# Yusheng-Xu/VGS-SVGS-Segmentation

Measured on AMD Instinct MI355X. Metric: segmented points/sec (end-to-end VGS), higher is better.
Workload: dtype f32

## Files before the change

include/vgs.h:

```cpp
#ifndef VGS_H_
#define VGS_H_

#include <stdint.h>

#ifdef __cplusplus
extern "C" {
#endif

typedef enum {
  VGS_OK = 0,
  VGS_E_ARG = 1,
  VGS_E_STATE = 2,
  VGS_E_HIP = 3,
  VGS_E_NOMEM = 4,
  VGS_E_UNSUPPORTED = 5,
  VGS_E_IO = 6,
  VGS_E_PEER = 7
} vgs_status;

typedef struct {
  int32_t method;
  float voxel_size;
  float graph_size;
  float sig_p, sig_n, sig_o, sig_e, sig_c, sig_w;
// ... 55 lines not shown
vgs_status vgs_adjacency(vgs_ctx* ctx);
vgs_status vgs_segment(vgs_ctx* ctx);
vgs_status vgs_run(vgs_ctx* ctx);

vgs_status svgs_set_supervoxel_labels(vgs_ctx* ctx, const int32_t* labels_host, int32_t max_label);
vgs_status svgs_supervoxels(vgs_ctx* ctx);
vgs_status svgs_segment(vgs_ctx* ctx);
vgs_status svgs_get_supervoxel_labels(vgs_ctx* ctx, int32_t* labels, int32_t* max_label);

vgs_status vgs_get_counts(vgs_ctx* ctx, int64_t* counts );
vgs_status vgs_get_stage_times(vgs_ctx* ctx, double* ms );
vgs_status vgs_get_schedule_counters(vgs_ctx* ctx, int64_t* out );
vgs_status vgs_get_schedule_counters_ex(vgs_ctx* ctx, int64_t* out, int32_t n);
vgs_status vgs_screen_table(const vgs_params* params, float* d2_stop, float* ctab_scale, float* ctab );
vgs_status vgs_get_bbox(vgs_ctx* ctx, double* min3_max3);
vgs_status vgs_get_voxel_table(vgs_ctx* ctx, uint32_t* key, int32_t* start, int32_t* point_idx);
vgs_status vgs_get_voxel_centers(vgs_ctx* ctx, float* center3V);
vgs_status vgs_get_point_voxel(vgs_ctx* ctx, int32_t* voxel_of_point );
vgs_status vgs_get_attributes(vgs_ctx* ctx, float* centroid, float* normal, float* eigen8, uint8_t* used);
vgs_status vgs_get_lists(vgs_ctx* ctx, int32_t which, int64_t* offsets, int32_t* idx);
enum { VGS_ORDER_VOXEL_ID = 0, VGS_ORDER_REFERENCE = 1 };
vgs_status vgs_get_lists_ordered(vgs_ctx* ctx, int32_t which, int32_t order, int64_t* offsets, int32_t* idx);
vgs_status vgs_get_adjacency_counts(vgs_ctx* ctx, int32_t* n_all );
vgs_status vgs_get_local_weights(vgs_ctx* ctx, int32_t node_id, int32_t* n, int32_t* ids, float* weights);
vgs_status vgs_get_node_labels(vgs_ctx* ctx, int32_t* component_root ,
                               int32_t* kept_label );
vgs_status vgs_get_point_labels(vgs_ctx* ctx, int32_t* labels );
vgs_status vgs_get_point_labels_async(vgs_ctx* ctx, int32_t* labels);
vgs_status vgs_wait_point_labels(vgs_ctx* ctx);
vgs_status vgs_get_point_labels_device(vgs_ctx* ctx, const int32_t** labels_dev );
vgs_status vgs_get_clusters(vgs_ctx* ctx, int64_t* offsets, int32_t* point_idx);
vgs_status vgs_get_clusters_ordered(vgs_ctx* ctx, int32_t order, int64_t* offsets, int32_t* point_idx);
vgs_status vgs_get_clusters_device(vgs_ctx* ctx, const int64_t** offsets_dev, const int32_t** point_idx_dev);
vgs_status vgs_get_segment_descriptors(vgs_ctx* ctx, int64_t* n_points, int32_t* n_nodes, float* bbox6, double* centroid3, double* cov6,
                                       double* evals3, double* evecs9, float* eigen8);
vgs_status vgs_get_segment_descriptors_device(vgs_ctx* ctx, const int64_t** n_points, const int32_t** n_nodes, const float** bbox6,
                                              const double** centroid3, const double** cov6, const double** evals3, const double** evecs9,
                                              const float** eigen8);
vgs_status vgs_get_own_segment_moments(vgs_ctx* ctx, int64_t K, int64_t* n_records, int32_t* label, int64_t* n_points, int32_t* n_nodes,
                                       float* bbox6, float* anchor3, double* s9);
vgs_status vgs_segment_descriptors_from_moments(vgs_ctx* ctx, int64_t K, const int64_t* n_points, const int32_t* n_nodes, const float* bbox6,
                                                const float* anchor3, const double* s9, int64_t* n_points_out, int32_t* n_nodes_out,
                                                float* bbox6_out, double* centroid3, double* cov6, double* evals3, double* evecs9, float* eigen8);
enum { VGS_BOX_PRINCIPAL = 0, VGS_BOX_UPRIGHT = 1 };
vgs_status vgs_get_segment_boxes(vgs_ctx* ctx, int32_t frame, double* center3, double* half3, double* frame9, double* lo3, double* hi3);
vgs_status vgs_get_segment_boxes_device(vgs_ctx* ctx, int32_t frame, const double** center3, const double** half3, const double** frame9,
// ... 35 lines not shown
```

vgs-svgs-segmentation_amd/_lib.py:

```python
from __future__ import annotations

import ctypes as C
import os
import subprocess

_HERE = os.path.dirname(os.path.abspath(__file__))
LIB_PATH = os.path.join(_HERE, os.path.basename(os.environ.get("VGS_LIB", "libvgs_hip.so")))
CSRC = os.path.join(_HERE, "csrc")

VGS_OK, VGS_E_ARG, VGS_E_STATE, VGS_E_HIP, VGS_E_NOMEM, VGS_E_UNSUPPORTED, VGS_E_IO, VGS_E_PEER = range(8)
STATUS_NAMES = ["VGS_OK", "VGS_E_ARG", "VGS_E_STATE", "VGS_E_HIP", "VGS_E_NOMEM", "VGS_E_UNSUPPORTED", "VGS_E_IO", "VGS_E_PEER"]

N_POINTS, N_FINITE, N_VOXELS, N_USED, N_ADJ, N_CLUSTERS, N_KEPT, N_PAIRS, N_DEPTH, N_ISOLATED, N_REATTACHED, N_SUPERVOXELS = range(12)
N_COUNTS = 16
T_VOXELIZE, T_FEATURES, T_ADJACENCY, T_LOCALCUT, T_MERGE, T_LABELS, T_TOTAL, T_LOCALCUT_KERNEL, T_SUPERVOXEL = range(9)
T_COUNT = 12


class VgsParams(C.Structure):
    _fields_ = [
        ("method", C.c_int32), ("voxel_size", C.c_float), ("graph_size", C.c_float),
        ("sig_p", C.c_float), ("sig_n", C.c_float), ("sig_o", C.c_float), ("sig_e", C.c_float), ("sig_c", C.c_float),
        ("sig_w", C.c_float), ("cut_thred", C.c_float),
        ("points_min", C.c_int32), ("adjacency_min", C.c_int32), ("voxels_min", C.c_int32),
# ... 31 lines not shown
    ("vgs_host_unregister", C.c_int, [_P]),
    ("vgs_voxelize", C.c_int, [_P]),
    ("vgs_features", C.c_int, [_P]),
    ("vgs_adjacency", C.c_int, [_P]),
    ("vgs_segment", C.c_int, [_P]),
    ("vgs_run", C.c_int, [_P]),
    ("svgs_set_supervoxel_labels", C.c_int, [_P, _P, C.c_int32]),
    ("svgs_supervoxels", C.c_int, [_P]),
    ("svgs_segment", C.c_int, [_P]),
    ("svgs_get_supervoxel_labels", C.c_int, [_P, _P, C.POINTER(C.c_int32)]),
    ("vgs_get_counts", C.c_int, [_P, _P]),
    ("vgs_get_schedule_counters", C.c_int, [_P, _P]),
    ("vgs_get_schedule_counters_ex", C.c_int, [_P, _P, C.c_int32]),
    ("vgs_screen_table", C.c_int, [_P, _P, _P, _P]),
    ("vgs_get_stage_times", C.c_int, [_P, _P]),
    ("vgs_get_bbox", C.c_int, [_P, _P]),
    ("vgs_get_voxel_table", C.c_int, [_P, _P, _P, _P]),
    ("vgs_get_voxel_centers", C.c_int, [_P, _P]),
    ("vgs_get_point_voxel", C.c_int, [_P, _P]),
    ("vgs_get_attributes", C.c_int, [_P, _P, _P, _P, _P]),
    ("vgs_get_lists", C.c_int, [_P, C.c_int32, _P, _P]),
    ("vgs_get_lists_ordered", C.c_int, [_P, C.c_int32, C.c_int32, _P, _P]),
    ("vgs_get_adjacency_counts", C.c_int, [_P, _P]),
    ("vgs_get_local_weights", C.c_int, [_P, C.c_int32, C.POINTER(C.c_int32), _P, _P]),
    ("vgs_get_node_labels", C.c_int, [_P, _P, _P]),
    ("vgs_get_point_labels", C.c_int, [_P, _P]),
    ("vgs_get_point_labels_async", C.c_int, [_P, _P]),
    ("vgs_wait_point_labels", C.c_int, [_P]),
    ("vgs_get_point_labels_device", C.c_int, [_P, C.POINTER(_P)]),
    ("vgs_get_clusters", C.c_int, [_P, _P, _P]),
    ("vgs_get_clusters_ordered", C.c_int, [_P, C.c_int32, _P, _P]),
    ("vgs_get_clusters_device", C.c_int, [_P, _P, _P]),
    ("vgs_get_segment_descriptors", C.c_int, [_P, _P, _P, _P, _P, _P, _P, _P, _P]),
    ("vgs_get_segment_descriptors_device", C.c_int, [_P, _P, _P, _P, _P, _P, _P, _P, _P]),
    ("vgs_get_own_segment_moments", C.c_int, [_P, C.c_int64, _P, _P, _P, _P, _P, _P, _P]),
    ("vgs_segment_descriptors_from_moments", C.c_int, [_P, C.c_int64, _P, _P, _P, _P, _P, _P, _P, _P, _P, _P, _P, _P, _P]),
    ("vgs_get_segment_boxes", C.c_int, [_P, C.c_int32, _P, _P, _P, _P, _P]),
    ("vgs_get_segment_boxes_device", C.c_int, [_P, C.c_int32, _P, _P, _P, _P, _P]),
    ("vgs_get_own_segment_extents", C.c_int, [_P, C.c_int64, C.c_int32, _P, _P, _P, _P, _P, _P, _P]),
    ("vgs_segment_boxes_from_extents", C.c_int, [_P, C.c_int64, C.c_int32, _P, _P, _P, _P, _P, _P, _P, _P]),
    ("vgs_get_segment_graph", C.c_int, [_P, _P, _P, _P, _P, _P, _P, _P, _P]),
    ("vgs_get_segment_graph_device", C.c_int, [_P, _P, _P, _P, _P, _P, _P, _P, _P]),
    ("vgs_set_halo_labels", C.c_int, [_P, _P, _P, C.c_int64]),
    ("vgs_get_own_segment_graph", C.c_int, [_P, C.c_int64, _P, _P, _P, _P, _P, _P, _P, _P]),
    ("vgs_grid_state_init", C.c_int, [C.POINTER(VgsGridState)]),
    ("vgs_grid_advance", C.c_int, [_P, C.POINTER(VgsGridState)]),
# ... 38 lines not shown
```

vgs-svgs-segmentation_amd/api.py:

```python
from __future__ import annotations

import ctypes as C

import numpy as np

from . import _lib
from ._lib import VgsError, VgsGridState, VgsParams


def default_params(method=2, **kw):
    p = VgsParams()
    L = _lib.lib()
    (L.vgs_params_default_svgs if method == 3 else L.vgs_params_default_vgs)(C.byref(p))
    for k, v in kw.items():
        if not hasattr(p, k):
            raise AttributeError(k)
        setattr(p, k, v)
    return p


def parse_task_file(path):
    p = VgsParams()
    a = C.create_string_buffer(512)
    b = C.create_string_buffer(512)
# ... 142 lines not shown
        cen = np.zeros((V, 3), dtype=np.float32)
        nrm = np.zeros((V, 3), dtype=np.float32)
        eig = np.zeros((V, 8), dtype=np.float32)
        used = np.zeros(V, dtype=np.uint8)
        self._ck(self._L.vgs_get_attributes(self._h, _ptr(cen), _ptr(nrm), _ptr(eig), _ptr(used)))
        return dict(centroid=cen, normal=nrm, eigen=eig, used=used)

    LISTS = {"adjacency": 0, "connect_cut": 1, "connect_cross": 2, "connect_final": 3}

    def lists(self, which, order="voxel_id"):
        V = self.counts()["voxels"]
        off = np.zeros(V + 1, dtype=np.int64)
        w, o = self.LISTS[which], self.ORDERS[order]
        self._ck(self._L.vgs_get_lists_ordered(self._h, w, o, _ptr(off), None))
        idx = np.zeros(max(int(off[-1]), 1), dtype=np.int32)
        self._ck(self._L.vgs_get_lists_ordered(self._h, w, o, _ptr(off), _ptr(idx)))
        return off, idx[:int(off[-1])]

    def adjacency_counts(self):
        out = np.zeros(self.counts()["voxels"], dtype=np.int32)
        self._ck(self._L.vgs_get_adjacency_counts(self._h, _ptr(out)))
        return out

    def local_weights(self, node_id):
        n = C.c_int32(0)
        self._ck(self._L.vgs_get_local_weights(self._h, int(node_id), C.byref(n), None, None))
        ids = np.zeros(max(n.value, 1), dtype=np.int32)
        W = np.zeros((max(n.value, 1), max(n.value, 1)), dtype=np.float32)
        if n.value:
            self._ck(self._L.vgs_get_local_weights(self._h, int(node_id), C.byref(n), _ptr(ids), _ptr(W)))
        return ids[:n.value], W[:n.value, :n.value]

    def node_labels(self):
        V = self.counts()["voxels"]
        root = np.zeros(V, dtype=np.int32)
        kept = np.zeros(V, dtype=np.int32)
        self._ck(self._L.vgs_get_node_labels(self._h, _ptr(root), _ptr(kept)))
        return root, kept

    def point_labels(self):
        out = np.zeros(self.n, dtype=np.int32)
        self._ck(self._L.vgs_get_point_labels(self._h, _ptr(out)))
        return out

    def supervoxel_labels(self):
        out = np.zeros(self.n, dtype=np.int32)
# ... 283 lines not shown
```

vgs-svgs-segmentation_amd/csrc/adjacency.hip:

```cpp
#include <algorithm>
#include <cstdio>
#include <cstdlib>
#include <vector>

#include "vgs_context.hpp"

#include "brick_table.hpp"

template <int CAP, bool FULL>
__global__ __launch_bounds__(64) void k_adjacency(const uint64_t* __restrict__ vox_code, const uint32_t* __restrict__ used_ids,
                                                  int64_t U, const Brick* __restrict__ bricks,
                                                  uint32_t hbits, const int32_t* __restrict__ offsets, int n_off, int R, int depth,
                                                  float res_f, float min_x, float min_y, float min_z, float r2,
                                                  const NodeRec* __restrict__ node, int adj_stride,
                                                  uint64_t* __restrict__ adj_key, uint32_t* __restrict__ adj_cnt,
                                                  uint32_t* __restrict__ adj_mused, uint16_t* __restrict__ gtab, int gstride, int ngroups,
                                                  const int32_t* __restrict__ nvals, const uint32_t* __restrict__ redo, unsigned int* __restrict__ n_redo,
                                                  uint32_t* __restrict__ redo_out, uint16_t* __restrict__ adj_off, unsigned int* __restrict__ n_redo_out) {
  __shared__ uint64_t lst[CAP];
  __shared__ uint8_t gl[CAP];
  __shared__ uint16_t loff[CAP];
  __shared__ float ctab[3][32];
  const int lane = threadIdx.x;
  auto do_row = [&](const int64_t u) {
// ... 454 lines not shown
    row[first + rank] = key;
    if (orow) orow[first + rank] = loff[p];
  }
  if (lane == 0) { adj_cnt[u] = (uint32_t)cnt; adj_mused[u] = (uint32_t)mused; }
  if (gtab) {
    uint16_t* gt = gtab + (int64_t)u * gstride;
    for (int r = lane; r <= ngroups; r += 64) {
      const int g = r < ngroups ? (nvals[r] & 255) : 0;
      gt[r] = (uint16_t)(r < ngroups ? ((s_hist[g >> 1] >> (16 * (g & 1))) & 0xffffu) : (uint32_t)cnt);
    }
  }
  };
  if constexpr (LISTED) {
    for (unsigned int w = blockIdx.x; w < *n_rows_in; w += gridDim.x) {
      do_row((int64_t)rows_in[w]);
      __syncthreads();
    }
  } else {
    const int64_t u = vgs_xcd_item(blockIdx.x, U);
    if (u < U) do_row(u);
  }
}

bool vgs_unused_are_inert(const vgs_params& p) {
  VgsWeightParams W;
  W.inv_sig_p = 1.0f / p.sig_p; W.inv_sig_n = 1.0f / p.sig_n; W.inv_sig_o = 1.0f / p.sig_o;
  W.inv_sig_e = 1.0f / p.sig_e; W.inv_sig_c = 1.0f / p.sig_c;
  W.inv_sig_w2 = 1.0f / (p.sig_w * p.sig_w);
  W.svgs = (p.method == 3) ? 1 : 0;
  const float d100[5] = {100.f, 100.f, 100.f, 100.f, 100.f};
  const float w_dead = vm_distance_weight(d100, W);
  return !(w_dead > vm_cut_threshold(1.0f, p.cut_thred, 1));
}

static vgs_status build_hash_and_offsets(vgs_ctx* c, float* r2_out) {
  if (!c->bricks_ready) {
    vgs_status bs = vgs_build_bricks(c, c->node.p);
    if (bs != VGS_OK) return bs;
  }
  c->bricks_ready = false;
  const double r = (double)c->P.graph_size;
  const double res = (double)c->P.voxel_size;
  *r2_out = (float)(r * r);
  if (c->adj_tab_valid && c->adj_tab_graph == c->P.graph_size && c->adj_tab_voxel == c->P.voxel_size) return VGS_OK;
  c->adj_tab_valid = false;
  const int R = (int)std::ceil(r / res) + 1;
  if (R > 127) { c->err = "graph_size / voxel_size > 126 voxels"; return VGS_E_UNSUPPORTED; }
  std::vector<std::pair<int, int32_t>> offs;
  const double lim2 = (r / res) * (r / res) * (1.0 + 1e-4) + 1e-3;
  for (int dz = -R; dz <= R; ++dz)
    for (int dy = -R; dy <= R; ++dy)
      for (int dx = -R; dx <= R; ++dx) {
        const int d2 = dx * dx + dy * dy + dz * dz;
        if ((double)d2 <= lim2) offs.emplace_back(d2, (int32_t)((dx & 0xff) | ((dy & 0xff) << 8) | ((dz & 0xff) << 16)));
      }
  std::sort(offs.begin(), offs.end());
  c->n_off = (int)offs.size();
  c->adj_R = R;
  {
    int Rm = 0;
    for (const auto& o : offs) {
      const int32_t pk = o.second;
      const int d[3] = {(int)(int8_t)(pk & 0xff), (int)(int8_t)((pk >> 8) & 0xff), (int)(int8_t)((pk >> 16) & 0xff)};
      for (int a = 0; a < 3; ++a) Rm = std::max(Rm, std::abs(d[a]));
    }
    const int Bh = (Rm + 3) / 4, NB = 2 * Bh + 1, NB3 = NB * NB * NB;
    c->adj_mask_nb = 0;
    if (NB == 3 || NB == 5 || NB == 7) {
      std::vector<uint64_t> masks((size_t)64 * NB3, 0ull);
      for (int p = 0; p < 64; ++p) {
        const int px = p & 3, py = (p >> 2) & 3, pz = p >> 4;
        for (const auto& o : offs) {
          const int32_t pk = o.second;
          const int dx = (int)(int8_t)(pk & 0xff), dy = (int)(int8_t)((pk >> 8) & 0xff), dz = (int)(int8_t)((pk >> 16) & 0xff);
          const int ax = px + dx, ay = py + dy, az = pz + dz;
          const int bi = (ax >= 0 ? ax / 4 : -((3 - ax) / 4)), bj = (ay >= 0 ? ay / 4 : -((3 - ay) / 4)), bk = (az >= 0 ? az / 4 : -((3 - az) / 4));
          const int lx = ax - 4 * bi, ly = ay - 4 * bj, lz = az - 4 * bk;
          const int local = (lz & 1) | ((ly & 1) << 1) | ((lx & 1) << 2) | ((lz & 2) << 2) | ((ly & 2) << 3) | ((lx & 2) << 4);
          masks[(size_t)p * NB3 + (size_t)(((bk + Bh) * NB + (bj + Bh)) * NB + (bi + Bh))] |= 1ull << local;
        }
      }
      VGS_HIP_TRY(c, c->adj_masks.ensure(masks.size()));
      VGS_HIP_TRY(c, hipMemcpy(c->adj_masks.p, masks.data(), masks.size() * 8, hipMemcpyHostToDevice));
      c->adj_mask_nb = NB;
    }
  }
  std::vector<int32_t> packed(offs.size());
  for (size_t k = 0; k < offs.size(); ++k) packed[k] = offs[k].second;
  {
    int Rm = 0;
    for (const auto& o : offs) {
      const int32_t pk = o.second;
      Rm = std::max(Rm, std::max(std::abs((int)(int8_t)(pk & 0xff)), std::max(std::abs((int)(int8_t)((pk >> 8) & 0xff)), std::abs((int)(int8_t)((pk >> 16) & 0xff)))));
    }
    c->cb_R = Rm;
    const int D = 2 * Rm + 1;
    c->cb_words = (D * D * D + 31) / 32;
  }
  VGS_HIP_TRY(c, c->offsets.ensure(packed.size()));
  VGS_HIP_TRY(c, hipMemcpy(c->offsets.p, packed.data(), packed.size() * sizeof(int32_t), hipMemcpyHostToDevice));
  c->adj_stride = c->n_off;
  std::vector<int32_t> nvals;
  std::vector<uint8_t> nrank(256, 0xff);
  for (const auto& o : offs)
// ... 14 lines not shown
vgs_status vgs_run_adjacency(vgs_ctx* c, bool full, uint64_t* out_key, uint32_t* out_cnt, uint32_t* out_nall, float r2, const uint32_t* ids,
                             int64_t n_ids) {
  const int64_t U = ids ? n_ids : c->U;
  const uint32_t* row_ids = ids ? ids : c->used_ids.p;
  const float res_f = c->P.voxel_size;
  const float mnx = (float)c->box.min[0], mny = (float)c->box.min[1], mnz = (float)c->box.min[2];
  uint16_t* gt = nullptr;
  uint16_t* off = nullptr;
  if (out_key == c->adj_key.p && c->adj_have_gtab) {
    VGS_HIP_TRY(c, c->adj_gtab.ensure((size_t)U * c->adj_gstride));
    gt = c->adj_gtab.p;
  }
  if (out_key == c->adj_key.p && c->P.method == 2 && c->adj_R <= 15) {
    VGS_HIP_TRY(c, c->adj_off.ensure((size_t)U * c->adj_stride));
    off = c->adj_off.p;
  }
  c->adj_have_off = (out_key == c->adj_key.p) ? (off != nullptr) : c->adj_have_off;
#define LAUNCH_ADJ(CAPV, FULLV, GRID, REDO, NREDO, REDO_OUT)                                                                 \
  hipLaunchKernelGGL((k_adjacency<CAPV, FULLV>), dim3(GRID), dim3(64), 0, c->stream, c->vox_code.p, row_ids, U,            \
                     (const Brick*)c->hkey.p, c->hbits, c->offsets.p, c->n_off, c->adj_R, c->box.depth, res_f, mnx, mny, mnz, r2, c->node.p, \
                     c->adj_stride, out_key, out_cnt, out_nall, gt, c->adj_gstride, c->adj_ngroups, c->adj_nvals.p, REDO, NREDO, REDO_OUT, off, NREDO)
  if (2 * c->adj_R + 1 > 32) { c->err = "neighbour ball wider than 31 voxels (graph_size / voxel_size > ~12)"; return VGS_E_UNSUPPORTED; }
  if (c->n_off <= 1024 && !full && c->adj_mask_nb > 0 && gt && !c->K.no_adjmasks) {
    VGS_HIP_TRY(c, c->work_ids.ensure(2 * (size_t)U + 16)); VGS_HIP_TRY(c, c->counters.ensure(64));
    unsigned int* d_nredo = (unsigned int*)(c->counters.p + 40);
    VGS_HIP_TRY(c, hipMemsetAsync(d_nredo, 0, 8, c->stream));
#define LAUNCH_ADJM(NBV)                                                                                                          \
    hipLaunchKernelGGL((k_adjacency_masks<240, NBV, 5>), dim3(vgs_xcd_grid(U)), dim3(64), 0, c->stream, c->vox_code.p, row_ids, U,  \
                       (const Brick*)c->hkey.p, c->hbits, c->adj_masks.p, c->adj_R, res_f, mnx, mny, mnz, r2, c->adj_stride, out_key,     \
                       out_cnt, out_nall, gt, c->adj_gstride, c->adj_ngroups, c->adj_nvals.p, d_nredo, c->work_ids.p, off)
    if (c->adj_mask_nb == 3) LAUNCH_ADJM(3); else LAUNCH_ADJM(5);
#undef LAUNCH_ADJM
    unsigned int* d_nredo2 = d_nredo + 1;
    uint32_t* list2 = c->work_ids.p + U;
    const unsigned int g2 = (unsigned int)(U < 2048 ? U : 2048);
#define LAUNCH_ADJM2(NBV)                                                                                                         \
    hipLaunchKernelGGL((k_adjacency_masks<512, NBV, 9, true>), dim3(g2), dim3(64), 0, c->stream, c->vox_code.p, row_ids, U,          \
                       (const Brick*)c->hkey.p, c->hbits, c->adj_masks.p, c->adj_R, res_f, mnx, mny, mnz, r2, c->adj_stride, out_key,     \
                       out_cnt, out_nall, gt, c->adj_gstride, c->adj_ngroups, c->adj_nvals.p, d_nredo2, list2, off,                      \
                       (const uint32_t*)c->work_ids.p, (const unsigned int*)d_nredo)
    if (c->adj_mask_nb == 3) LAUNCH_ADJM2(3); else LAUNCH_ADJM2(5);
#undef LAUNCH_ADJM2
    LAUNCH_ADJ(1024, false, g2, list2, d_nredo2, nullptr);
  } else if (c->n_off <= 8192 && !full && c->adj_mask_nb == 7 && gt && !c->K.no_adjmasks) {
    VGS_HIP_TRY(c, c->work_ids.ensure(2 * (size_t)U + 16)); VGS_HIP_TRY(c, c->counters.ensure(64));
    unsigned int* d_n1 = (unsigned int*)(c->counters.p + 40);
    unsigned int* d_n2 = (unsigned int*)(c->counters.p + 41);
    VGS_HIP_TRY(c, hipMemsetAsync(d_n1, 0, 16, c->stream));
    uint32_t* list1 = c->work_ids.p;
    uint32_t* list2 = c->work_ids.p + U;
    hipLaunchKernelGGL((k_adjacency_masks<512, 7, 13>), dim3(vgs_xcd_grid(U)), dim3(64), 0, c->stream, c->vox_code.p, row_ids, U,
                       (const Brick*)c->hkey.p, c->hbits, c->adj_masks.p, c->adj_R, res_f, mnx, mny, mnz, r2, c->adj_stride, out_key,
                       out_cnt, out_nall, gt, c->adj_gstride, c->adj_ngroups, c->adj_nvals.p, d_n1, list1, off);
    const unsigned int g2 = (unsigned int)(U < 4096 ? U : 4096);
    hipLaunchKernelGGL((k_adjacency<2048, false>), dim3(g2), dim3(64), 0, c->stream, c->vox_code.p, row_ids, U, (const Brick*)c->hkey.p, c->hbits,
// ... 6 lines not shown
    if (full) LAUNCH_ADJ(1024, true, vgs_xcd_grid(U), nullptr, nullptr, nullptr); else LAUNCH_ADJ(1024, false, vgs_xcd_grid(U), nullptr, nullptr, nullptr);
  } else if (c->n_off <= 8192) {
    VGS_HIP_TRY(c, c->work_ids.ensure((size_t)U + 16)); VGS_HIP_TRY(c, c->counters.ensure(64));
    unsigned int* d_nredo = (unsigned int*)(c->counters.p + 40);
    VGS_HIP_TRY(c, hipMemsetAsync(d_nredo, 0, 4, c->stream));
    if (full) LAUNCH_ADJ(2048, true, vgs_xcd_grid(U), nullptr, d_nredo, c->work_ids.p); else LAUNCH_ADJ(2048, false, vgs_xcd_grid(U), nullptr, d_nredo, c->work_ids.p);
    const unsigned int g2 = (unsigned int)(U < 4096 ? U : 4096);
    if (full) LAUNCH_ADJ(8192, true, g2, c->work_ids.p, d_nredo, nullptr); else LAUNCH_ADJ(8192, false, g2, c->work_ids.p, d_nredo, nullptr);
  }
  else { c->err = "neighbour ball larger than 8192 lattice offsets (graph_size / voxel_size > ~12)"; return VGS_E_UNSUPPORTED; }
#undef LAUNCH_ADJ
  VGS_HIP_TRY(c, hipGetLastError());
  return VGS_OK;
}

vgs_status vgs_stage_adjacency(vgs_ctx* c) {
  const int64_t V = c->V, U = c->U;
  c->counts[VGS_N_ADJ] = 0;
  if (V == 0) return VGS_OK;
  float r2 = 0.f;
  vgs_status st = build_hash_and_offsets(c, &r2);
  if (st != VGS_OK) return st;
  c->adj_r2 = r2;
  if (U == 0) return VGS_OK;
  c->adj_pruned = vgs_unused_are_inert(c->P);
  {
    const double fixed_rows = (double)U * ((double)(c->cb_words > 0 && c->cb_words <= VGS_CB_MAX_WORDS ? c->cb_words : 0) * 4.0 + (double)c->adj_gstride * 2.0 + 16.0 * 4.0 + 32.0)
                              + (double)V * (16.0 * 16.0 + 8.0 + 10.0);
    const double need = (double)U * (double)c->adj_stride * 12.0 + fixed_rows;
    const double held = (double)c->adj_key.cap * 8.0 + (double)c->adj_off.cap * 2.0 + (double)c->conn.cap + (double)c->conn_bits.cap * 4.0 +
                        (double)c->adj_gtab.cap * 2.0 + (double)c->work_ids.cap * 4.0 + (double)c->nl_ent.cap * 16.0 + (double)c->pl_state.cap;
    size_t free_b = 0, total_b = 0;
    VGS_HIP_TRY(c, hipMemGetInfo(&free_b, &total_b));
    if (need > held + (double)free_b * 0.97) {
      char msg[512];
      snprintf(msg, sizeof(msg), "adjacency / connect tables need %.1f GB (%lld used voxels x %d lattice offsets of a search ball of %.1f voxels x 12 B, + per-voxel lists) "
               "but %.1f GB are free on the device (%.1f GB in all): lower graph_size / voxel_size, or split the cloud into spatial tiles (include/vgs_tiles.h)",
               need / 1e9, (long long)U, c->adj_stride, (double)(c->P.graph_size / c->P.voxel_size), ((double)free_b + held) / 1e9, (double)total_b / 1e9);
      c->err = msg;
      return VGS_E_NOMEM;
    }
  }
  VGS_HIP_TRY(c, c->adj_key.ensure((size_t)U * c->adj_stride));
  VGS_HIP_TRY(c, c->adj_cnt.ensure(U)); VGS_HIP_TRY(c, c->adj_mused.ensure(U));
  st = vgs_run_adjacency(c, !c->adj_pruned, c->adj_key.p, c->adj_cnt.p, c->adj_mused.p, r2);
  if (st != VGS_OK) return st;
// ... 3 lines not shown
```

vgs-svgs-segmentation_amd/csrc/capi.hip:

```cpp
#include <algorithm>
#include <cstdio>
#include <cstdlib>
#include <cstring>
#include <fstream>
#include <string>
#include <vector>

#include <dlfcn.h>

#include "vgs_context.hpp"

static thread_local std::string g_create_err;

static const char* const VGS_STAGE_NAMES[VGS_T_COUNT] = {"vgs:voxelize", "vgs:features", "vgs:adjacency", "vgs:localcut", "vgs:merge", "vgs:labels",
                                                         "vgs:total", "vgs:localcut_kernel", "vgs:supervoxels", "vgs:localcut_bulk", "", ""};
struct RoctxApi {
  int (*push)(const char*) = nullptr;
  int (*pop)() = nullptr;
  RoctxApi() {
    for (const char* name : {"librocprofiler-sdk-roctx.so.1", "librocprofiler-sdk-roctx.so", "libroctx64.so.4", "libroctx64.so"}) {
      void* h = dlopen(name, RTLD_LAZY | RTLD_LOCAL);
      if (!h) continue;
      push = (int (*)(const char*))dlsym(h, "roctxRangePushA");
      pop = (int (*)())dlsym(h, "roctxRangePop");
// ... 155 lines not shown
            hipEventCreateWithFlags(&c->ev_ho2, hipEventDisableTiming) == hipSuccess;
  for (int i = 0; ok && i < 16; ++i) ok = hipEventCreate(&c->ev[i]) == hipSuccess;
  for (int i = 0; ok && i < VGS_T_COUNT; ++i) ok = hipEventCreate(&c->tev[i][0]) == hipSuccess && hipEventCreate(&c->tev[i][1]) == hipSuccess;
  if (!ok) { g_create_err = "vgs_create: hipStreamCreate/hipEventCreate failed"; vgs_destroy(c); return VGS_E_HIP; }
  vgs_read_env_knobs(c);
  *out = c;
  return VGS_OK;
}

void vgs_destroy(vgs_ctx* c) {
  if (!c) return;
  (void)hipSetDevice(c->device);
  if (c->stream) (void)hipStreamSynchronize(c->stream);
  if (c->stream2) (void)hipStreamSynchronize(c->stream2);
  if (c->stream3) (void)hipStreamSynchronize(c->stream3);
  if (c->stream4) (void)hipStreamSynchronize(c->stream4);
  if (c->s_h2d) (void)hipStreamSynchronize(c->s_h2d);
  if (c->s_d2h) (void)hipStreamSynchronize(c->s_d2h);
  c->xyz_buf[0].release(); c->xyz_buf[1].release(); c->pt_label_alt.release(); c->grow_state.release();
  c->code_a.release(); c->code_b.release(); c->perm_a.release(); c->perm_b.release(); c->sort_tmp.release();
  c->head_flag.release(); c->pt_vox.release(); c->vox_tile.release(); c->vox_code.release(); c->vox_start.release();
  c->xs.release(); c->ys.release(); c->zs.release();
  c->node.release(); c->used_ids.release(); c->used_rank.release();
  c->hkey.release(); c->hval.release(); c->offsets.release(); c->adj_masks.release(); c->adj_gtab.release(); c->adj_nvals.release(); c->adj_nrank.release(); c->adj_key.release(); c->adj_off.release(); c->adj_cnt.release(); c->adj_mused.release();
  c->nl_cnt.release(); c->nl_tot.release(); c->nl_ent.release(); c->lc_ctab.release(); c->pl_state.release(); c->pl_ent.release(); c->pl_work.release();
  c->sd_key.release(); c->sd_ids.release(); c->sd_vp.release(); c->sd_seg.release(); c->sd_tmp.release(); c->sd_part.release();
  c->sd_npts.release(); c->sd_nnodes.release(); c->sd_bbox.release(); c->sd_eig8.release(); c->sd_cen.release(); c->sd_cov.release(); c->sd_eval.release(); c->sd_evec.release();
  c->sd_apos.release(); c->sd_mom.release();
  c->sb_part.release(); c->sbt_in.release(); c->sbt_frame.release(); c->sbt_out.release(); c->sbt_idx.release();
  for (int f = 0; f < 2; ++f) { c->sb_frame[f].release(); c->sb_lo[f].release(); c->sb_hi[f].release(); c->sb_half[f].release(); c->sb_center[f].release(); }
  c->sg_lab.release(); c->sg_nrec.release(); c->sg_ridx.release(); c->sg_ework.release(); c->sg_meta.release(); c->sg_roff.release(); c->sg_rkey.release(); c->sg_rec.release(); c->sg_part.release(); c->sg_tmp.release();
  c->sg_ab.release(); c->sg_nodes.release(); c->sg_npairs.release(); c->sg_nfin.release(); c->sg_wsum.release(); c->sg_wmin.release(); c->sg_wmax.release();
  c->cl_off.release(); c->cl_idx.release(); c->conn.release(); c->evals.release(); c->lc_pending.release(); c->lc_defer.release(); c->lc_defer_flag.release(); c->csize.release(); c->attach.release(); c->cc_flags.release(); c->parent.release(); c->csz.release();
  c->vc_cen.release(); c->vc_nrm.release(); c->vc_dist.release(); c->vc_state.release(); c->vc_tile_start.release(); c->vc_cell.release(); c->vc_plive.release(); c->vc_tile_of.release(); c->vc_tchg.release(); c->vc_nbr_tiles.release(); c->vc_halo.release(); c->vc_tile_meta.release(); c->vc_pool.release(); c->vc_ring.release(); c->vc_dbg.release(); c->vc_label.release();
  c->vc_seedkey.release(); c->vc_sums.release(); c->vc_count.release(); c->vc_accu.release(); c->vc_alive.release();
  c->sv_label.release(); c->sv_key_a.release(); c->sv_key_b.release(); c->cell_code_a.release(); c->cell_code_b.release();
  c->cell_id_a.release(); c->cell_id_b.release(); c->cell_start.release();
  c->owned.release(); c->straddle.release(); c->mixsrc.release(); c->bnd_code.release(); c->bnd_root.release(); c->root_label.release();
  c->bnd_code2.release(); c->bnd_root2.release(); c->bnd_cnt.release(); c->broot.release();
  c->kept_rank.release(); c->vox_label.release(); c->pt_label.release(); c->counters.release(); c->work_ids.release();
  if (c->pin) (void)hipHostFree(c->pin);
  for (int i = 0; i < 16; ++i) if (c->ev[i]) (void)hipEventDestroy(c->ev[i]);
  for (int i = 0; i < VGS_T_COUNT; ++i) for (int k = 0; k < 2; ++k) if (c->tev[i][k]) (void)hipEventDestroy(c->tev[i][k]);
  if (c->stream) (void)hipStreamDestroy(c->stream);
  if (c->stream2) (void)hipStreamDestroy(c->stream2);
  if (c->stream3) (void)hipStreamDestroy(c->stream3);
  if (c->stream4) (void)hipStreamDestroy(c->stream4);
// ... 438 lines not shown
  int64_t o = 0;
  for (int64_t v = 0; v < V; ++v) {
    offsets[v] = o;
    if (idx) std::memcpy(idx + o, L[v].data(), L[v].size() * 4);
    o += (int64_t)L[v].size();
  }
  offsets[V] = o;
  return VGS_OK;
}

vgs_status vgs_get_adjacency_counts(vgs_ctx* c, int32_t* n_all) {
  if (!c || !n_all) return VGS_E_ARG;
  if (c->stage < ST_ADJACENCY) { c->err = "vgs_get_adjacency_counts: adjacency first"; return VGS_E_STATE; }
  for (int64_t v = 0; v < c->V; ++v) n_all[v] = 0;
  if (c->U == 0) return VGS_OK;
  VGS_HIP_TRY(c, hipSetDevice(c->device));
  std::vector<uint32_t> ids((size_t)c->U), cnt((size_t)c->U);
  VGS_HIP_TRY(c, hipMemcpy(ids.data(), c->used_ids.p, ids.size() * 4, hipMemcpyDeviceToHost));
  VGS_HIP_TRY(c, hipMemcpy(cnt.data(), c->adj_mused.p, cnt.size() * 4, hipMemcpyDeviceToHost));
  for (int64_t u = 0; u < c->U; ++u) n_all[ids[u]] = (int32_t)cnt[u];
  return VGS_OK;
}

vgs_status vgs_get_node_labels(vgs_ctx* c, int32_t* root, int32_t* kept_label) {
  if (!c) return VGS_E_ARG;
  if (c->stage < ST_SEGMENTED) { c->err = "vgs_get_node_labels: segment first"; return VGS_E_STATE; }
  if (c->V == 0) return VGS_OK;
  if (root) VGS_HIP_TRY(c, hipMemcpy(root, c->parent.p, (size_t)c->V * 4, hipMemcpyDeviceToHost));
  if (kept_label) VGS_HIP_TRY(c, hipMemcpy(kept_label, c->vox_label.p, (size_t)c->V * 4, hipMemcpyDeviceToHost));
  return VGS_OK;
}

vgs_status vgs_get_point_labels(vgs_ctx* c, int32_t* labels) {
  if (!c || !labels) return VGS_E_ARG;
  if (c->stage < ST_SEGMENTED) { c->err = "vgs_get_point_labels: segment first"; return VGS_E_STATE; }
  { vgs_status se = vgs_ensure_point_labels(c); if (se != VGS_OK) return se; }
  if (c->N > 0) VGS_HIP_TRY(c, hipMemcpy(labels, c->pt_label.p, (size_t)c->N * 4, hipMemcpyDeviceToHost));
  return VGS_OK;
}

vgs_status vgs_get_point_labels_async(vgs_ctx* c, int32_t* labels) {
  if (!c || !labels) return VGS_E_ARG;
  if (c->stage < ST_SEGMENTED) { c->err = "vgs_get_point_labels_async: segment first"; return VGS_E_STATE; }
  VGS_HIP_TRY(c, hipSetDevice(c->device));
  if (c->d2h_open) { VGS_HIP_TRY(c, hipEventSynchronize(c->ev_d2h)); c->d2h_open = false; }
  if (c->N == 0) return VGS_OK;
// ... 90 lines not shown
```

vgs-svgs-segmentation_amd/csrc/vgs_context.hpp:

```cpp
#ifndef VGS_CONTEXT_HPP_
#define VGS_CONTEXT_HPP_

#include <hip/hip_runtime.h>
#include <stdint.h>
#include <string.h>

#include <string>
#include <vector>

#include "../../include/vgs.h"
#include "vgs_math.h"
#include "pairlist.hpp"

typedef VgsNode NodeRec;
static_assert(sizeof(NodeRec) == 64, "NodeRec must be 64 bytes");

#ifdef __HIPCC__
__device__ __forceinline__ int64_t vgs_xcd_item(unsigned int b, int64_t n) {
  const int64_t per = (n + 7) >> 3;
  return (int64_t)(b & 7u) * per + (int64_t)(b >> 3);
}
#endif
static inline unsigned int vgs_xcd_grid(int64_t n) { return (unsigned int)(((n + 7) >> 3) << 3); }

// ... 132 lines not shown
  DevBuf<uint64_t> hkey;
  DevBuf<uint32_t> hval;
  uint32_t hbits = 0;
  DevBuf<int32_t> offsets;
  DevBuf<uint64_t> adj_masks;
  int adj_mask_nb = 0;
  bool adj_tab_valid = false;
  float adj_tab_graph = 0.f, adj_tab_voxel = 0.f;
  DevBuf<uint16_t> adj_gtab;
  DevBuf<int32_t> adj_nvals;
  DevBuf<uint8_t> adj_nrank;
  int adj_ngroups = 0, adj_gstride = 0;
  bool adj_have_gtab = false;
  int n_off = 0;
  int adj_R = 0;
  int adj_stride = 0;
  DevBuf<uint64_t> adj_key;
  DevBuf<uint16_t> adj_off;
  bool adj_have_off = false;
  DevBuf<uint32_t> conn_bits;
  int cb_words = 0, cb_R = 0;
  bool cb_enabled = false;
  DevBuf<uint32_t> adj_cnt, adj_mused;
  bool adj_pruned = false;
  float adj_r2 = 0.f;

  DevBuf<uint8_t> nl_cnt;
  DevBuf<uint32_t> nl_tot;
  DevBuf<float4> nl_ent;
  bool nl_enabled = false;
  int nl_reach_steps = 0;
  bool nl_direct = false;

  DevBuf<uint8_t> pl_state;
  DevBuf<float4> pl_ent;
  DevBuf<uint32_t> pl_work;
  bool pl_enabled = false;
  bool pl_enabled_at_launch = false;
  hipEvent_t ev_ho = nullptr, ev_ho2 = nullptr;
  float pl_w_ring = 0.0f;

  DevBuf<uint8_t> conn;
  DevBuf<uint32_t> evals;
  DevBuf<uint8_t> lc_pending;
  DevBuf<uint8_t> lc_defer_flag;
  DevBuf<uint32_t> lc_defer;
// ... 177 lines not shown
```

Baseline: 1.623 billion.

## Group adjacency rows by shared brick to reuse neighbourhood occupancy in LDS

```diff
diff --git a/include/vgs.h b/include/vgs.h
--- a/include/vgs.h
+++ b/include/vgs.h
@@ -101,6 +101,7 @@
 enum { VGS_ORDER_VOXEL_ID = 0, VGS_ORDER_REFERENCE = 1 };
 vgs_status vgs_get_lists_ordered(vgs_ctx* ctx, int32_t which, int32_t order, int64_t* offsets, int32_t* idx);
 vgs_status vgs_get_adjacency_counts(vgs_ctx* ctx, int32_t* n_all );
+vgs_status vgs_get_adjacency_rows(vgs_ctx* ctx, int64_t* dims, uint64_t* keys, uint32_t* cnt, uint32_t* n_all, uint16_t* off, uint16_t* gtab);
 vgs_status vgs_get_local_weights(vgs_ctx* ctx, int32_t node_id, int32_t* n, int32_t* ids, float* weights);
 vgs_status vgs_get_node_labels(vgs_ctx* ctx, int32_t* component_root ,
                                int32_t* kept_label );
diff --git a/vgs-svgs-segmentation_amd/_lib.py b/vgs-svgs-segmentation_amd/_lib.py
--- a/vgs-svgs-segmentation_amd/_lib.py
+++ b/vgs-svgs-segmentation_amd/_lib.py
@@ -77,6 +77,7 @@
     ("vgs_get_lists", C.c_int, [_P, C.c_int32, _P, _P]),
     ("vgs_get_lists_ordered", C.c_int, [_P, C.c_int32, C.c_int32, _P, _P]),
     ("vgs_get_adjacency_counts", C.c_int, [_P, _P]),
+    ("vgs_get_adjacency_rows", C.c_int, [_P, _P, _P, _P, _P, _P, _P]),
     ("vgs_get_local_weights", C.c_int, [_P, C.c_int32, C.POINTER(C.c_int32), _P, _P]),
     ("vgs_get_node_labels", C.c_int, [_P, _P, _P]),
     ("vgs_get_point_labels", C.c_int, [_P, _P]),
diff --git a/vgs-svgs-segmentation_amd/api.py b/vgs-svgs-segmentation_amd/api.py
--- a/vgs-svgs-segmentation_amd/api.py
+++ b/vgs-svgs-segmentation_amd/api.py
@@ -188,6 +188,20 @@
         self._ck(self._L.vgs_get_adjacency_counts(self._h, _ptr(out)))
         return out
 
+    def adjacency_rows(self):
+        d = np.zeros(8, dtype=np.int64)
+        self._ck(self._L.vgs_get_adjacency_rows(self._h, _ptr(d), None, None, None, None, None))
+        U, stride, gstride, ngroups, have_off = (int(x) for x in d[:5])
+        keys = np.zeros((U, stride), dtype=np.uint64)
+        cnt = np.zeros(U, dtype=np.uint32)
+        n_all = np.zeros(U, dtype=np.uint32)
+        off = np.zeros((U, stride), dtype=np.uint16) if have_off else None
+        gtab = np.zeros((U, gstride), dtype=np.uint16) if gstride else None
+        if U:
+            self._ck(self._L.vgs_get_adjacency_rows(self._h, _ptr(d), _ptr(keys), _ptr(cnt), _ptr(n_all),
+                                                    _ptr(off) if have_off else None, _ptr(gtab) if gstride else None))
+        return dict(keys=keys, cnt=cnt, n_all=n_all, off=off, gtab=None if gtab is None else gtab[:, :ngroups + 1], runs=int(d[5]))
+
     def local_weights(self, node_id):
         n = C.c_int32(0)
         self._ck(self._L.vgs_get_local_weights(self._h, int(node_id), C.byref(n), None, None))
diff --git a/vgs-svgs-segmentation_amd/csrc/adjacency.hip b/vgs-svgs-segmentation_amd/csrc/adjacency.hip
--- a/vgs-svgs-segmentation_amd/csrc/adjacency.hip
+++ b/vgs-svgs-segmentation_amd/csrc/adjacency.hip
@@ -500,6 +500,261 @@
   }
 }
 
+#ifndef ADJB_WAVES
+#define ADJB_WAVES 4
+#endif
+#define ADJB_GRID 8192u
+
+__global__ __launch_bounds__(256) void k_brick_runs(const uint64_t* __restrict__ vox_code, const uint32_t* __restrict__ used_ids, int64_t U,
+                                                    uint2* __restrict__ runs, unsigned int* __restrict__ n_runs) {
+  const int64_t u = (int64_t)blockIdx.x * blockDim.x + threadIdx.x;
+  const int lane = threadIdx.x & 63;
+  bool head = false;
+  uint32_t len = 0;
+  if (u < U) {
+    const uint64_t b = vox_code[used_ids[u]] >> 6;
+    head = u == 0 || (vox_code[used_ids[u - 1]] >> 6) != b;
+    if (head) {
+      len = 1;
+      while (u + len < U && (vox_code[used_ids[u + len]] >> 6) == b) ++len;
+    }
+  }
+  const unsigned long long m = __ballot(head);
+  if (m == 0ull) return;
+  unsigned int base = 0;
+  if (lane == __ffsll((long long)m) - 1) base = atomicAdd(n_runs, (unsigned int)__popcll(m));
+  base = (unsigned int)__shfl((int)base, __ffsll((long long)m) - 1, 64);
+  if (head) runs[base + (unsigned int)__popcll(m & ((1ull << lane) - 1ull))] = make_uint2((uint32_t)u, len);
+}
+
+__device__ __forceinline__ void adjb_wave_sync() {
+  __builtin_amdgcn_fence(__ATOMIC_ACQ_REL, "workgroup");
+  __builtin_amdgcn_wave_barrier();
+}
+
+template <int CAP, int NB, int ADJM_TRIPS, int NW>
+__global__ __launch_bounds__(64 * NW) __attribute__((amdgpu_waves_per_eu(NB == 3 ? 8 : 7))) void k_adjacency_bricks(const uint64_t* __restrict__ vox_code, const uint32_t* __restrict__ used_ids,
+                                                              const uint2* __restrict__ runs, const unsigned int* __restrict__ n_runs,
+                                                              unsigned int* __restrict__ n_runs_keep,
+                                                              const Brick* __restrict__ bricks, uint32_t hbits, const uint64_t* __restrict__ masks,
+                                                              int R, float res_f, float min_x, float min_y, float min_z, float r2,
+                                                              int adj_stride, uint64_t* __restrict__ adj_key, uint32_t* __restrict__ adj_cnt,
+                                                              uint32_t* __restrict__ adj_mused, uint16_t* __restrict__ gtab, int gstride, int ngroups,
+                                                              const int32_t* __restrict__ nvals, unsigned int* __restrict__ n_redo,
+                                                              uint32_t* __restrict__ redo_out, uint16_t* __restrict__ adj_off) {
+  constexpr int NB3 = NB * NB * NB, Bh = NB / 2, CAPC = 64 * ADJM_TRIPS;
+  constexpr int BTRIPS = (NB3 + 63) / 64, ADJM_BRICKS = 64 * BTRIPS;
+  constexpr int ADJM_BRICKS_P2 = ADJM_BRICKS <= 64 ? 64 : (ADJM_BRICKS <= 128 ? 128 : (ADJM_BRICKS <= 256 ? 256 : 512));
+  static_assert(NB3 <= 512, "brick slot: nine bits of a candidate");
+  __shared__ uint64_t s_occ[ADJM_BRICKS];
+  __shared__ uint64_t s_used[ADJM_BRICKS];
+  __shared__ uint32_t s_first[ADJM_BRICKS];
+  constexpr int ROW_BYTES = CAP * 8 + CAP * 2 + CAP, SLOT_BYTES = ADJM_BRICKS * 8;
+  constexpr int BUF_BYTES = ((ROW_BYTES > SLOT_BYTES ? ROW_BYTES : SLOT_BYTES) + 15) & ~15;
+  struct WaveTabs {
+    __attribute__((aligned(16))) unsigned char buf[BUF_BYTES];
+    uint32_t hist[128], cur[128];
+    float ctab[3][32];
+    uint16_t pref[ADJM_BRICKS];
+  };
+  __shared__ WaveTabs s_w[NW];
+  const int tid = threadIdx.x, wave = __builtin_amdgcn_readfirstlane(tid >> 6);
+  WaveTabs& wt = s_w[wave];
+  uint16_t* const s_pref = wt.pref;
+  unsigned char* const s_buf = wt.buf;
+  uint64_t* const s_cm = (uint64_t*)s_buf;
+  uint64_t* const lst = (uint64_t*)s_buf;
+  uint16_t* const loff = (uint16_t*)(s_buf + CAP * 8);
+  uint8_t* const gl = s_buf + CAP * 8 + CAP * 2;
+  uint32_t* const s_hist = wt.hist;
+  uint32_t* const s_cur = wt.cur;
+  float (*const ctab)[32] = wt.ctab;
+  auto do_row = [&](const int64_t u) {
+  int lane = tid & 63;
+  asm volatile("" : "+v"(lane));
+  const uint32_t i = used_ids[u];
+  const uint64_t code = vox_code[i];
+  const uint32_t kx = vm_compact21(code >> 2), ky = vm_compact21(code >> 1), kz = vm_compact21(code);
+  const float cx = vm_voxel_center(kx, res_f, min_x), cy = vm_voxel_center(ky, res_f, min_y), cz = vm_voxel_center(kz, res_f, min_z);
+  if (lane < 2 * R + 1) {
+    ctab[0][lane] = vm_voxel_center(kx + (uint32_t)(lane - R), res_f, min_x);
+    ctab[1][lane] = vm_voxel_center(ky + (uint32_t)(lane - R), res_f, min_y);
+    ctab[2][lane] = vm_voxel_center(kz + (uint32_t)(lane - R), res_f, min_z);
+  }
+  for (int k = lane; k < 128; k += 64) s_hist[k] = 0;
+  const int px = (int)(kx & 3u), py = (int)(ky & 3u), pz = (int)(kz & 3u);
+  const uint64_t* mrow = masks + (size_t)((pz * 4 + py) * 4 + px) * (size_t)NB3;
+  uint64_t cand[BTRIPS];
+#pragma unroll
+  for (int trip = 0; trip < BTRIPS; ++trip) {
+    const int sidx = trip * 64 + lane;
+    cand[trip] = sidx < NB3 ? (s_occ[sidx] & mrow[sidx]) : 0ull;
+  }
+  int mine = 0;
+#pragma unroll
+  for (int trip = 0; trip < BTRIPS; ++trip) mine += __popcll(cand[trip]);
+  int incl = mine;
+  for (int o = 1; o < 64; o <<= 1) { const int v = __shfl_up(incl, o, 64); if (lane >= o) incl += v; }
+  const int ntot = __shfl(incl, 63, 64);
+  auto to_redo = [&]() { if (lane == 0) redo_out[atomicAdd(n_redo, 1u)] = (uint32_t)u; };
+  if (ntot > CAPC) { to_redo(); return; }
+  {
+    int pos = incl - mine;
+#pragma unroll
+    for (int trip = 0; trip < BTRIPS; ++trip) {
+      s_pref[lane * BTRIPS + trip] = (uint16_t)pos;
+      pos += __popcll(cand[trip]);
+      s_cm[trip * 64 + lane] = cand[trip];
+    }
+  }
+  adjb_wave_sync();
+  const float res2 = res_f * res_f;
+  int nstore = 0, mused = 0;
+  bool in_band = true;
+  uint64_t rkey[ADJM_TRIPS];
+  int rnorm[ADJM_TRIPS];
+#pragma unroll
+  for (int tr = 0; tr < ADJM_TRIPS; ++tr) {
+    rnorm[tr] = -1; rkey[tr] = 0;
+    const int q = tr * 64 + lane;
+    if (tr * 64 < ntot) {
+      bool keep = false, is_used = false;
+      if (q < ntot) {
+        int j = 0;
+#pragma unroll
+        for (int step = ADJM_BRICKS_P2 / 2; step >= 1; step >>= 1) {
+          const int mid = j + step;
+          if (mid < ADJM_BRICKS && (int)s_pref[mid] <= q) j = mid;
+        }
+        const int sidx = (j % BTRIPS) * 64 + j / BTRIPS;
+        int kth = q - (int)s_pref[j];
+        const uint64_t cmask = s_cm[sidx];
+        uint32_t w = (uint32_t)cmask;
+        int bit = 0;
+        { const int c = __popc(w); if (kth >= c) { kth -= c; w = (uint32_t)(cmask >> 32); bit = 32; } }
+        { const int c = __popc(w & 0xffffu); if (kth >= c) { kth -= c; w >>= 16; bit += 16; } }
+        { const int c = __popc(w & 0xffu); if (kth >= c) { kth -= c; w >>= 8; bit += 8; } }
+        { const int c = __popc(w & 0xfu); if (kth >= c) { kth -= c; w >>= 4; bit += 4; } }
+        { const int c = __popc(w & 0x3u); if (kth >= c) { kth -= c; w >>= 2; bit += 2; } }
+        { const int c = (int)(w & 1u); if (kth >= c) { bit += 1; } }
+        is_used = ((s_used[sidx] >> bit) & 1ull) != 0ull;
+        const int bi = sidx % NB - Bh, bj = (sidx / NB) % NB - Bh, bk = sidx / (NB * NB) - Bh;
+        const int lx = ((bit >> 2) & 1) | (((bit >> 5) & 1) << 1), ly = ((bit >> 1) & 1) | (((bit >> 4) & 1) << 1), lz = (bit & 1) | (((bit >> 3) & 1) << 1);
+        const int dx = 4 * bi + lx - px, dy = 4 * bj + ly - py, dz = 4 * bk + lz - pz;
+        const uint64_t occ = s_occ[sidx];
+        const uint64_t above = (bit == 63) ? 0ull : (occ >> (bit + 1));
+        const uint32_t t = s_first[sidx] + (uint32_t)__popcll(above);
+        const float tx = cx - ctab[0][dx + R];
+        const float ty = cy - ctab[1][dy + R];
+        const float tz = cz - ctab[2][dz + R];
+        const float d2 = (tx * tx + ty * ty) + tz * tz;
+        if (d2 < r2) {
+          keep = true;
+          const int norm = dx * dx + dy * dy + dz * dz;
+          in_band = in_band && (fabsf(d2 - (float)norm * res2) < 0.49f * res2) && (norm < 256);
+          if (is_used) {
+            rkey[tr] = ((uint64_t)vm_bits(d2) << 32) | t;
+            rnorm[tr] = (norm & 255) | (int)(((uint32_t)(dx + 16) | ((uint32_t)(dy + 16) << 5) | ((uint32_t)(dz + 16) << 10)) << 8);
+            atomicAdd(&s_hist[(norm & 255) >> 1], 1u << (16 * (norm & 1)));
+          }
+        }
+      }
+      nstore += __popcll(__ballot(keep && is_used));
+      mused += __popcll(__ballot(keep));
+    }
+  }
+  if (nstore > CAP || __ballot(!in_band) != 0ull) { to_redo(); return; }
+  adjb_wave_sync();
+  {
+    const uint32_t w0 = s_hist[2 * lane], w1 = s_hist[2 * lane + 1];
+    const uint32_t h[4] = {w0 & 0xffffu, w0 >> 16, w1 & 0xffffu, w1 >> 16};
+    const uint32_t sum = h[0] + h[1] + h[2] + h[3];
+    uint32_t inc = sum;
+    for (int o = 1; o < 64; o <<= 1) { const uint32_t v = (uint32_t)__shfl_up((int)inc, o, 64); if (lane >= o) inc += v; }
+    const uint32_t s0 = inc - sum, s1 = s0 + h[0], s2 = s1 + h[1], s3 = s2 + h[2];
+    const uint32_t p0 = s0 | (s1 << 16), p1 = s2 | (s3 << 16);
+    s_hist[2 * lane] = p0; s_hist[2 * lane + 1] = p1;
+    s_cur[2 * lane] = p0; s_cur[2 * lane + 1] = p1;
+  }
+  adjb_wave_sync();
+#pragma unroll
+  for (int tr = 0; tr < ADJM_TRIPS; ++tr) {
+    if (rnorm[tr] >= 0) {
+      const int g = rnorm[tr] & 255;
+      const uint32_t old = atomicAdd(&s_cur[g >> 1], 1u << (16 * (g & 1)));
+      const uint32_t pos = (old >> (16 * (g & 1))) & 0xffffu;
+      lst[pos] = rkey[tr]; gl[pos] = (uint8_t)g; loff[pos] = (uint16_t)(rnorm[tr] >> 8);
+    }
+  }
+  adjb_wave_sync();
+  uint64_t* row = adj_key + (int64_t)u * adj_stride;
+  uint16_t* orow = adj_off ? adj_off + (int64_t)u * adj_stride : nullptr;
+  const int cnt = nstore;
+  for (int p = lane; p < cnt; p += 64) {
+    const uint64_t key = lst[p];
+    const int g = gl[p];
+    const int first = (int)((s_hist[g >> 1] >> (16 * (g & 1))) & 0xffffu);
+    const int last = (int)((s_cur[g >> 1] >> (16 * (g & 1))) & 0xffffu);
+    int rank = 0;
+    for (int q = first; q < last; ++q) rank += lst[q] < key ? 1 : 0;
+    row[first + rank] = key;
+    if (orow) orow[first + rank] = loff[p];
+  }
+  if (lane == 0) { adj_cnt[u] = (uint32_t)cnt; adj_mused[u] = (uint32_t)mused; }
+  if (gtab) {
+    uint16_t* gt = gtab + (int64_t)u * gstride;
+    for (int r = lane; r <= ngroups; r += 64) {
+      const int g = r < ngroups ? (nvals[r] & 255) : 0;
+      gt[r] = (uint16_t)(r < ngroups ? ((s_hist[g >> 1] >> (16 * (g & 1))) & 0xffffu) : (uint32_t)cnt);
+    }
+  }
+  };
+  const unsigned int n = *n_runs;
+  if (blockIdx.x == 0 && tid == 0) *n_runs_keep = n;
+  const unsigned int per = (n + 7u) >> 3, xcd = blockIdx.x & 7u;
+  const uint64_t* const mall = masks + (size_t)64 * NB3;
+#pragma nounroll
+  for (unsigned int j = blockIdx.x >> 3; j < per; j += gridDim.x >> 3) {
+    const unsigned int w = xcd * per + j;
+    if (w >= n) break;
+    const uint2 run = runs[w];
+    {
+      const uint64_t code0 = vox_code[used_ids[run.x]];
+      const int bx = (int)(vm_compact21(code0 >> 2) >> 2), by = (int)(vm_compact21(code0 >> 1) >> 2), bz = (int)(vm_compact21(code0) >> 2);
+#pragma nounroll
+      for (int sidx = tid; sidx < NB3; sidx += 64 * NW) {
+        uint64_t occ = 0ull, usd = 0ull;
+        uint32_t first = 0u;
+        const int bi = sidx % NB - Bh, bj = (sidx / NB) % NB - Bh, bk = sidx / (NB * NB) - Bh;
+        const int nbx = bx + bi, nby = by + bj, nbz = bz + bk;
+        if (mall[sidx] != 0ull && nbx >= 0 && nby >= 0 && nbz >= 0) {
+          const unsigned long long key = (((unsigned long long)nbz << 42) | ((unsigned long long)nby << 21) | (unsigned long long)nbx) + 1ull;
+          const uint32_t mask = (1u << hbits) - 1u;
+          uint32_t sl = hash_slot(key, hbits);
+          while (true) {
+            const ulonglong2 k01 = *(const ulonglong2*)&bricks[sl];
+            if (k01.x == key) {
+              const ulonglong2 k23 = *((const ulonglong2*)&bricks[sl] + 1);
+              occ = k01.y; usd = k23.x; first = (uint32_t)k23.y;
+              break;
+            }
+            if (k01.x == 0ull) break;
+            sl = (sl + 1) & mask;
+          }
+        }
+        s_occ[sidx] = occ; s_used[sidx] = usd; s_first[sidx] = first;
+      }
+    }
+    __syncthreads();
+#pragma nounroll
+    for (uint32_t r = (uint32_t)wave; r < run.y; r += NW) {
+      do_row((int64_t)run.x + r);
+      adjb_wave_sync();
+    }
+    __syncthreads();
+  }
+}
+
 bool vgs_unused_are_inert(const vgs_params& p) {
   VgsWeightParams W;
   W.inv_sig_p = 1.0f / p.sig_p; W.inv_sig_n = 1.0f / p.sig_n; W.inv_sig_o = 1.0f / p.sig_o;
@@ -545,7 +800,7 @@
     const int Bh = (Rm + 3) / 4, NB = 2 * Bh + 1, NB3 = NB * NB * NB;
     c->adj_mask_nb = 0;
     if (NB == 3 || NB == 5 || NB == 7) {
-      std::vector<uint64_t> masks((size_t)64 * NB3, 0ull);
+      std::vector<uint64_t> masks((size_t)65 * NB3, 0ull);
       for (int p = 0; p < 64; ++p) {
         const int px = p & 3, py = (p >> 2) & 3, pz = p >> 4;
         for (const auto& o : offs) {
@@ -558,6 +813,8 @@
           masks[(size_t)p * NB3 + (size_t)(((bk + Bh) * NB + (bj + Bh)) * NB + (bi + Bh))] |= 1ull << local;
         }
       }
+      for (int p = 0; p < 64; ++p)
+        for (int b = 0; b < NB3; ++b) masks[(size_t)64 * NB3 + (size_t)b] |= masks[(size_t)p * NB3 + (size_t)b];
       VGS_HIP_TRY(c, c->adj_masks.ensure(masks.size()));
       VGS_HIP_TRY(c, hipMemcpy(c->adj_masks.p, masks.data(), masks.size() * 8, hipMemcpyHostToDevice));
       c->adj_mask_nb = NB;
@@ -618,15 +875,30 @@
                      c->adj_stride, out_key, out_cnt, out_nall, gt, c->adj_gstride, c->adj_ngroups, c->adj_nvals.p, REDO, NREDO, REDO_OUT, off, NREDO)
   if (2 * c->adj_R + 1 > 32) { c->err = "neighbour ball wider than 31 voxels (graph_size / voxel_size > ~12)"; return VGS_E_UNSUPPORTED; }
   if (c->n_off <= 1024 && !full && c->adj_mask_nb > 0 && gt && !c->K.no_adjmasks) {
-    VGS_HIP_TRY(c, c->work_ids.ensure(2 * (size_t)U + 16)); VGS_HIP_TRY(c, c->counters.ensure(64));
+    VGS_HIP_TRY(c, c->work_ids.ensure(4 * (size_t)U + 32)); VGS_HIP_TRY(c, c->counters.ensure(64)); VGS_HIP_TRY(c, c->adj_nruns.ensure(2));
     unsigned int* d_nredo = (unsigned int*)(c->counters.p + 40);
-    VGS_HIP_TRY(c, hipMemsetAsync(d_nredo, 0, 8, c->stream));
-#define LAUNCH_ADJM(NBV)                                                                                                          \
-    hipLaunchKernelGGL((k_adjacency_masks<240, NBV, 5>), dim3(vgs_xcd_grid(U)), dim3(64), 0, c->stream, c->vox_code.p, row_ids, U,  \
-                       (const Brick*)c->hkey.p, c->hbits, c->adj_masks.p, c->adj_R, res_f, mnx, mny, mnz, r2, c->adj_stride, out_key,     \
-                       out_cnt, out_nall, gt, c->adj_gstride, c->adj_ngroups, c->adj_nvals.p, d_nredo, c->work_ids.p, off)
-    if (c->adj_mask_nb == 3) LAUNCH_ADJM(3); else LAUNCH_ADJM(5);
+    unsigned int* d_nruns = (unsigned int*)(c->counters.p + 41);
+    VGS_HIP_TRY(c, hipMemsetAsync(d_nredo, 0, 16, c->stream));
+    if (!ids) {
+      uint2* runs = (uint2*)(c->work_ids.p + 2 * (((size_t)U + 7) & ~(size_t)7) + 16);
+      hipLaunchKernelGGL(k_brick_runs, dim3((unsigned)((U + 255) / 256)), dim3(256), 0, c->stream, c->vox_code.p, row_ids, U, runs, d_nruns);
+      const unsigned int gb = std::min(vgs_xcd_grid(U), ADJB_GRID);
+#define LAUNCH_ADJB(NBV)                                                                                                                       \
+      hipLaunchKernelGGL((k_adjacency_bricks<240, NBV, 5, ADJB_WAVES>), dim3(gb), dim3(64 * ADJB_WAVES), 0, c->stream, c->vox_code.p, row_ids,  \
+                         (const uint2*)runs, (const unsigned int*)d_nruns, c->adj_nruns.p, (const Brick*)c->hkey.p, c->hbits, c->adj_masks.p,  \
+                         c->adj_R, res_f, mnx, mny, mnz, r2, c->adj_stride, out_key, out_cnt, out_nall, gt, c->adj_gstride, c->adj_ngroups,     \
+                         c->adj_nvals.p, d_nredo, c->work_ids.p, off)
+      if (c->adj_mask_nb == 3) LAUNCH_ADJB(3); else LAUNCH_ADJB(5);
+#undef LAUNCH_ADJB
+      c->adj_runs_valid = true;
+    } else {
+#define LAUNCH_ADJM(NBV)                                                                                                            \
+      hipLaunchKernelGGL((k_adjacency_masks<240, NBV, 5>), dim3(vgs_xcd_grid(U)), dim3(64), 0, c->stream, c->vox_code.p, row_ids, U,  \
+                         (const Brick*)c->hkey.p, c->hbits, c->adj_masks.p, c->adj_R, res_f, mnx, mny, mnz, r2, c->adj_stride, out_key,   \
+                         out_cnt, out_nall, gt, c->adj_gstride, c->adj_ngroups, c->adj_nvals.p, d_nredo, c->work_ids.p, off)
+      if (c->adj_mask_nb == 3) LAUNCH_ADJM(3); else LAUNCH_ADJM(5);
 #undef LAUNCH_ADJM
+    }
     unsigned int* d_nredo2 = d_nredo + 1;
     uint32_t* list2 = c->work_ids.p + U;
     const unsigned int g2 = (unsigned int)(U < 2048 ? U : 2048);
@@ -679,6 +951,7 @@
   vgs_status st = build_hash_and_offsets(c, &r2);
   if (st != VGS_OK) return st;
   c->adj_r2 = r2;
+  c->adj_runs_valid = false;
   if (U == 0) return VGS_OK;
   c->adj_pruned = vgs_unused_are_inert(c->P);
   {
diff --git a/vgs-svgs-segmentation_amd/csrc/capi.hip b/vgs-svgs-segmentation_amd/csrc/capi.hip
--- a/vgs-svgs-segmentation_amd/csrc/capi.hip
+++ b/vgs-svgs-segmentation_amd/csrc/capi.hip
@@ -201,7 +201,7 @@
   c->head_flag.release(); c->pt_vox.release(); c->vox_tile.release(); c->vox_code.release(); c->vox_start.release();
   c->xs.release(); c->ys.release(); c->zs.release();
   c->node.release(); c->used_ids.release(); c->used_rank.release();
-  c->hkey.release(); c->hval.release(); c->offsets.release(); c->adj_masks.release(); c->adj_gtab.release(); c->adj_nvals.release(); c->adj_nrank.release(); c->adj_key.release(); c->adj_off.release(); c->adj_cnt.release(); c->adj_mused.release();
+  c->hkey.release(); c->hval.release(); c->offsets.release(); c->adj_masks.release(); c->adj_gtab.release(); c->adj_nvals.release(); c->adj_nrank.release(); c->adj_key.release(); c->adj_off.release(); c->adj_cnt.release(); c->adj_mused.release(); c->adj_nruns.release();
   c->nl_cnt.release(); c->nl_tot.release(); c->nl_ent.release(); c->lc_ctab.release(); c->pl_state.release(); c->pl_ent.release(); c->pl_work.release();
   c->sd_key.release(); c->sd_ids.release(); c->sd_vp.release(); c->sd_seg.release(); c->sd_tmp.release(); c->sd_part.release();
   c->sd_npts.release(); c->sd_nnodes.release(); c->sd_bbox.release(); c->sd_eig8.release(); c->sd_cen.release(); c->sd_cov.release(); c->sd_eval.release(); c->sd_evec.release();
@@ -686,6 +686,31 @@
   return VGS_OK;
 }
 
+vgs_status vgs_get_adjacency_rows(vgs_ctx* c, int64_t* dims, uint64_t* keys, uint32_t* cnt, uint32_t* n_all, uint16_t* off, uint16_t* gtab) {
+  if (!c || !dims) return VGS_E_ARG;
+  if (c->stage < ST_ADJACENCY) { c->err = "vgs_get_adjacency_rows: adjacency first"; return VGS_E_STATE; }
+  const size_t U = (size_t)c->U, stride = (size_t)c->adj_stride;
+  const bool have_gt = c->adj_have_gtab && c->adj_gtab.p && c->adj_gtab.cap >= U * (size_t)c->adj_gstride;
+  const bool have_off = c->adj_have_off && c->adj_off.p;
+  for (int k = 0; k < 8; ++k) dims[k] = 0;
+  dims[0] = (int64_t)U; dims[1] = (int64_t)stride; dims[2] = have_gt ? c->adj_gstride : 0; dims[3] = c->adj_ngroups; dims[4] = have_off ? 1 : 0;
+  dims[5] = -1;
+  if (U == 0) return VGS_OK;
+  VGS_HIP_TRY(c, hipSetDevice(c->device));
+  VGS_HIP_TRY(c, hipStreamSynchronize(c->stream));
+  if (c->adj_runs_valid) {
+    unsigned int n = 0;
+    VGS_HIP_TRY(c, hipMemcpy(&n, c->adj_nruns.p, 4, hipMemcpyDeviceToHost));
+    dims[5] = (int64_t)n;
+  }
+  if (keys) VGS_HIP_TRY(c, hipMemcpy(keys, c->adj_key.p, U * stride * 8, hipMemcpyDeviceToHost));
+  if (cnt) VGS_HIP_TRY(c, hipMemcpy(cnt, c->adj_cnt.p, U * 4, hipMemcpyDeviceToHost));
+  if (n_all) VGS_HIP_TRY(c, hipMemcpy(n_all, c->adj_mused.p, U * 4, hipMemcpyDeviceToHost));
+  if (off && have_off) VGS_HIP_TRY(c, hipMemcpy(off, c->adj_off.p, U * stride * 2, hipMemcpyDeviceToHost));
+  if (gtab && have_gt) VGS_HIP_TRY(c, hipMemcpy(gtab, c->adj_gtab.p, U * (size_t)c->adj_gstride * 2, hipMemcpyDeviceToHost));
+  return VGS_OK;
+}
+
 vgs_status vgs_get_node_labels(vgs_ctx* c, int32_t* root, int32_t* kept_label) {
   if (!c) return VGS_E_ARG;
   if (c->stage < ST_SEGMENTED) { c->err = "vgs_get_node_labels: segment first"; return VGS_E_STATE; }
diff --git a/vgs-svgs-segmentation_amd/csrc/vgs_context.hpp b/vgs-svgs-segmentation_amd/csrc/vgs_context.hpp
--- a/vgs-svgs-segmentation_amd/csrc/vgs_context.hpp
+++ b/vgs-svgs-segmentation_amd/csrc/vgs_context.hpp
@@ -178,6 +178,8 @@
   int cb_words = 0, cb_R = 0;
   bool cb_enabled = false;
   DevBuf<uint32_t> adj_cnt, adj_mused;
+  DevBuf<unsigned int> adj_nruns;
+  bool adj_runs_valid = false;
   bool adj_pruned = false;
   float adj_r2 = 0.f;
 
```

New measurement: 1.597 billion. 1.6% lower.
